# teamtomo/torch-motion-correction

Measured on AMD Instinct MI355X. Metric: frames/sec motion-corrected, 40×4k×4k fp32 stack, 1/2/4/8 MI355X, higher is better.
Workload: dtype f32; 1 GPU; 40-frame 4096x4096 fp32 movie, global rigid shift estimate+correct (estimate_global_motion -> correct_motion, frames + sum out), 1 stack per GPU per step, consecutive steps overlapped on two HIP streams; b_factor=500

## Files before the change

### torch_motion_correction_amd/csrc/mc_wave_fft.h

```cpp
#pragma once

#ifdef __HIPCC__
#include "mc_common.h"
#define MC_HD __host__ __device__ __forceinline__
#else
#include <math.h>
#include <stdint.h>
struct cfloat {
  float x, y;
};
#define MC_HD static inline
#endif

typedef float wf2 __attribute__((ext_vector_type(2)));

#define WF_N 2048
#define WF_SLAB 1024

MC_HD wf2 wf_make(float re, float im) { return wf2{re, im}; }
MC_HD wf2 wf_from(cfloat c) { return wf2{c.x, c.y}; }
MC_HD cfloat wf_to(wf2 v) { return cfloat{v.x, v.y}; }

MC_HD wf2 wf_add_mi(wf2 a, wf2 b) {
#if defined(__HIP_DEVICE_COMPILE__)
// ... 119 lines not shown
      a[4 * p + r] = a[4 * r + p];
      a[4 * r + p] = s;
    }
}

template <int KEEP>
MC_HD void wf_dft8_pruned(const wf2 (&e)[4], const wf2 (&o)[4], wf2 (&z)[8]) {
  const float H = 0.70710678118654752440f;
  wf2 e0 = e[0], e1 = e[1], e2 = e[2], e3 = e[3];
  wf2 o0 = o[0], o1 = o[1], o2 = o[2], o3 = o[3];
  wf_bfly4(e0, e1, e2, e3);
  wf_bfly4(o0, o1, o2, o3);
  z[0] = e0 + o0;
  z[7] = wf_fma_c(e3, o3, H, H);
  if (KEEP >= 2) {
    z[1] = wf_fma_c(e1, o1, H, -H);
    z[6] = wf_sub_mi(e2, o2);
  }
  if (KEEP >= 4) {
    z[2] = wf_add_mi(e2, o2);
    z[3] = wf_fma_c(e3, o3, -H, -H);
    z[4] = e0 - o0;
    z[5] = wf_fma_c(e1, o1, -H, H);
  }
}

struct WfLane {
  int x1w_base, x1w_mask;
  int x1r[4];
  int x2w;
  int x2r[4];
  int kbin[4];
  int self;
};

MC_HD WfLane wf_lane(int t) {
  WfLane L;
  {
    const int n2 = t >> 2, h1 = (t >> 1) & 1, h0 = t & 1;
    L.x1w_base = (n2 * 2 + h1) * 32 + h0 * 16;
    L.x1w_mask = (n2 & 3) | (h1 << 2) | (h0 << 3);
  }
  {
    const int k1 = t & 15, g2 = t >> 4, h1 = g2 >> 1, h0 = g2 & 1;
    const int lanepart = h1 * 32 + h0 * 16, lo = k1 ^ ((h1 << 2) | (h0 << 3));
    for (int v = 0; v < 4; ++v) L.x1r[v] = lanepart + (lo ^ v);
    L.x2w = g2 * 256 + k1;
  }
  L.kbin[0] = t;
  L.kbin[1] = t == 0 ? 128 : 256 - t;
  L.kbin[2] = 64 + t;
  L.kbin[3] = 192 - t;
  for (int s = 0; s < 4; ++s) L.x2r[s] = L.kbin[s];
  L.self = t == 0;
  return L;
}

MC_HD wf2 wf_unpack(wf2 zk, wf2 zmr, wf2 wk) {
  const wf2 zm = {zmr.x, -zmr.y};
  const wf2 sm = zk + zm, d = zk - zm;
  const wf2 wd = wf_cmul(d, wk);
  return wf_add_mi(sm, wd) * 0.5f;
}

template <int KEEP>
MC_HD void wf_unpack_lane(const wf2 (&z)[4][8], const wf2 (&wk)[4], bool self, wf2 (&X)[4][KEEP]) {
  const float C1 = 0.92387953251128673848f, S1 = 0.38268343236508978178f;
#pragma unroll
  for (int k3 = 0; k3 < KEEP; ++k3) {
    const wf2 m_a0 = self ? z[0][(8 - k3) & 7] : z[1][7 - k3];
    const wf2 m_a1 = self ? z[1][7 - k3] : z[0][7 - k3];
    wf2 w[4] = {wk[0], wk[1], wk[2], wk[3]};
    if (k3 == 1) {
#pragma unroll
      for (int s = 0; s < 4; ++s) w[s] = wf_cmulc(w[s], C1, -S1);
    }
    X[0][k3] = wf_unpack(z[0][k3], m_a0, w[0]);
    X[1][k3] = wf_unpack(z[1][k3], m_a1, w[1]);
    X[2][k3] = wf_unpack(z[2][k3], z[3][7 - k3], w[2]);
    X[3][k3] = wf_unpack(z[3][k3], z[2][7 - k3], w[3]);
  }
}

#define WF5_N 512
#define WF5_SLAB 512

MC_HD void wf_dft8(wf2 (&a)[8]) {
  const float H = 0.70710678118654752440f;
  wf2 e0 = a[0], e1 = a[2], e2 = a[4], e3 = a[6];
  wf2 o0 = a[1], o1 = a[3], o2 = a[5], o3 = a[7];
  wf_bfly4(e0, e1, e2, e3);
  wf_bfly4(o0, o1, o2, o3);
  a[0] = e0 + o0;
  a[4] = e0 - o0;
  a[1] = wf_fma_c(e1, o1, H, -H);
  a[5] = wf_fma_c(e1, o1, -H, H);
  a[2] = wf_add_mi(e2, o2);
  a[6] = wf_sub_mi(e2, o2);
  a[3] = wf_fma_c(e3, o3, -H, -H);
  a[7] = wf_fma_c(e3, o3, H, H);
}

MC_HD int wf5_x1(int k1, int n2, int n3) { return ((n2 * 8 + (k1 ^ n2)) * 8) + (n3 ^ (4 * (k1 >> 2))); }
MC_HD int wf5_x2(int k2, int n3, int k1) { return ((n3 * 8 + (k2 ^ n3)) * 8) + k1; }

#define WF10_N 1024
MC_HD int wf10_x1(int k1, int q) { return k1 * 64 + (q ^ ((2 * k1) & 31)); }
MC_HD int wf10_x2(int k1, int k2, int n3) { return n3 * 128 + k2 * 16 + k1; }

MC_HD void wf_twiddle8(wf2 (&a)[8], wf2 w1) {
  const wf2 w2 = wf_cmul(w1, w1), w3 = wf_cmul(w2, w1), w4 = wf_cmul(w2, w2);
  a[1] = wf_cmul(a[1], w1);
  a[2] = wf_cmul(a[2], w2);
  a[3] = wf_cmul(a[3], w3);
  a[4] = wf_cmul(a[4], w4);
  a[5] = wf_cmul(a[5], wf_cmul(w4, w1));
  a[6] = wf_cmul(a[6], wf_cmul(w4, w2));
  a[7] = wf_cmul(a[7], wf_cmul(w4, w3));
}
MC_HD void wf_twiddle16(wf2 (&a)[16], wf2 w1, wf2 w2, wf2 w4, wf2 w8) {
  const wf2 w3 = wf_cmul(w2, w1), w5 = wf_cmul(w4, w1), w6 = wf_cmul(w4, w2), w7 = wf_cmul(w4, w3);
  a[1] = wf_cmul(a[1], w1); a[2] = wf_cmul(a[2], w2); a[3] = wf_cmul(a[3], w3); a[4] = wf_cmul(a[4], w4);
  a[5] = wf_cmul(a[5], w5); a[6] = wf_cmul(a[6], w6); a[7] = wf_cmul(a[7], w7); a[8] = wf_cmul(a[8], w8);
  a[9] = wf_cmul(a[9], wf_cmul(w8, w1)); a[10] = wf_cmul(a[10], wf_cmul(w8, w2));
  a[11] = wf_cmul(a[11], wf_cmul(w8, w3)); a[12] = wf_cmul(a[12], wf_cmul(w8, w4));
  a[13] = wf_cmul(a[13], wf_cmul(w8, w5)); a[14] = wf_cmul(a[14], wf_cmul(w8, w6));
  a[15] = wf_cmul(a[15], wf_cmul(w8, w7));
}
```

### torch_motion_correction_amd/csrc/xc_fft.hip

```cpp
#include <stdlib.h>
#include <string.h>
#include <type_traits>
#include "xc_common.h"
#include "mc_wave_fft.h"




template <int LOGN, bool STATS, int RAW = 0>
__global__ __launch_bounds__(MC_WG) void xc_rows_fwd(
    const void* __restrict__ src_any, const int64_t* __restrict__ job_off, int64_t row_stride,
    const int* __restrict__ job_expo, const float* __restrict__ mask,
    const float* __restrict__ mean_rstd, cfloat* __restrict__ T1,
    const cfloat* __restrict__ tw_row, XcGeom g, XcBox box, double* __restrict__ stats_acc,
    const float* __restrict__ gain, const float* __restrict__ job_sub) {
  constexpr int N = 1 << LOGN;
  constexpr int NT = fft_threads(N), SG = MC_WG / NT;
  constexpr int R0 = FftPlan<N>::radix(0), NB0 = N / R0, IT0 = (NB0 + NT - 1) / NT;
  extern __shared__ __attribute__((aligned(16))) char smem[];
  const int tid = threadIdx.x;
  const int lt = tid & (NT - 1), sg = tid / NT;
  cfloat* l0 = reinterpret_cast<cfloat*>(smem) + sg * 2 * lds_len(N);
  cfloat* l1 = l0 + lds_len(N);
  cfloat* stg = reinterpret_cast<cfloat*>(smem) + SG * 2 * lds_len(N);
// ... 1169 lines not shown
    const cfloat* __restrict__ S_ref, const int* __restrict__ ref_idx, cfloat* __restrict__ T2n,
    float* __restrict__ bounds, const cfloat* __restrict__ tw_col, float scale, XcGeom g, int nstore) {
  constexpr int H = 1 << LOGH;
  __shared__ __attribute__((aligned(16))) cfloat line[R16 ? H : lds_len(H)];
  constexpr int NOUT = H / MC_WG;
  const int tid = threadIdx.x;
  const int p = blockIdx.y;
  const int nky = g.kyp + g.kyn;
  float acc[NOUT];
#pragma unroll
  for (int c = 0; c < NOUT; ++c) acc[c] = 0.f;
  const int64_t cur_base = (int64_t)cur_idx[p] * g.nkx, ref_base = (int64_t)ref_idx[p] * g.nkx;
  int kyi4[4];
  cfloat pc[4], pr[4];
  auto fetch4 = [&](int kx, cfloat (&c4)[4], cfloat (&r4)[4]) {
    const cfloat* cur = S_cur + (cur_base + kx) * nky;
    const cfloat* ref = S_ref + (ref_base + kx) * nky;
#pragma unroll
    for (int s4 = 0; s4 < 4; ++s4) {
      c4[s4] = kyi4[s4] >= 0 ? cur[kyi4[s4]] : cmake(0.f, 0.f);
      r4[s4] = kyi4[s4] >= 0 ? ref[kyi4[s4]] : cmake(0.f, 0.f);
    }
  };
  R16Tw TW;
  if constexpr (R16) {
    TW = r16_twiddles(tid, tw_col);
#pragma unroll
    for (int s4 = 0; s4 < 4; ++s4) kyi4[s4] = kept_index(tid + 256 * (s4 < 2 ? s4 : s4 + 12), H, g.kyp, g.kyn);
    if ((int)blockIdx.x * XC_NEAR_COLS < g.nkx) fetch4(blockIdx.x * XC_NEAR_COLS, pc, pr);
  }
#pragma unroll 1
  for (int cc = 0; cc < XC_NEAR_COLS; ++cc) {
    const int kx = blockIdx.x * XC_NEAR_COLS + cc;
    if (kx >= g.nkx) break;
    const cfloat* cur = S_cur + (cur_base + kx) * nky;
    const cfloat* ref = S_ref + (ref_base + kx) * nky;
    cfloat* outn = T2n + ((int64_t)p * g.nkx + kx) * (2 * nstore);
    const float wgt = kx == 0 ? 1.f : 2.f;
    auto load = [&](int ky) {
      const int kyi = kept_index(ky, H, g.kyp, g.kyn);
      if (kyi < 0) return cmake(0.f, 0.f);
      return cscale(cmulc(ref[kyi], cur[kyi]), scale);
    };
    cfloat qc[4], qr[4];
    if constexpr (R16) {
#pragma unroll
      for (int s4 = 0; s4 < 4; ++s4) {
        qc[s4] = pc[s4];
        qr[s4] = pr[s4];
      }
      if (cc + 1 < XC_NEAR_COLS && kx + 1 < g.nkx) fetch4(kx + 1, pc, pr);
    }
    auto load16 = [&](int n1, int) { return cscale(cmulc(qr[n1 < 2 ? n1 : n1 - 12], qc[n1 < 2 ? n1 : n1 - 12]), scale); };
    int c = 0;
    auto store = [&](int y, cfloat v) {
      const int yn = y < nstore ? y : y - (H - 2 * nstore);
      if (yn >= 0 && yn < 2 * nstore && (y < nstore || y >= H - nstore)) outn[yn] = v;
      acc[c++] += wgt * __builtin_amdgcn_sqrtf(v.x * v.x + v.y * v.y);
    };
    int tcol = tid;
    asm volatile("" : "+v"(tcol));
    __builtin_assume(tcol >= 0 && tcol < MC_WG);
    __builtin_assume(nstore > 0 && nstore <= 256);
    if constexpr (R16) wg_fft4096_r16_tw<+1, 2, 8>(line, tcol, TW, load16, store);
    else wg_fft<H, +1>(line, tcol, tw_col, 1, load, store);
    __syncthreads();
  }
  if constexpr (R16) {
#pragma unroll
    for (int k3 = 0; k3 < 16; ++k3) atomicAdd(&bounds[(int64_t)p * H + tid + 256 * k3], acc[k3]);
  } else {
    constexpr int R = (H >= 4096) ? 8 : (H == 2048 ? 4 : 2);
    constexpr int NB = H / R, IT = NB / MC_WG;
    static_assert(IT * R == NOUT, "row ownership of the last pass");
#pragma unroll
    for (int it = 0; it < IT; ++it)
#pragma unroll
      for (int m = 0; m < R; ++m)
        atomicAdd(&bounds[(int64_t)p * H + tid + it * MC_WG + m * NB], acc[it * R + m]);
  }
}

__global__ void xc_search_init(int* __restrict__ best, int* __restrict__ gate, float* __restrict__ bounds,
                               int npairs, int nbounds, float* __restrict__ shift_table, int nshift) {
  const int i = blockIdx.x * blockDim.x + threadIdx.x;
  if (i < nbounds) bounds[i] = 0.f;
  if (i < nshift) shift_table[i] = 0.f;
  if (i < npairs) best[i] = (int)0x807fffffu;
  if (i == 0) gate[0] = 0;
}

__global__ void xc_far_needed(const float* __restrict__ bounds, const int* __restrict__ best,
                              float* __restrict__ part_val, int* __restrict__ part_idx,
                              int* __restrict__ need_full, int H, int RG, int near) {
  const int ngrp = H / RG;
  const int p = blockIdx.y;
  const int grp = near + blockIdx.x * blockDim.x + threadIdx.x;
  if (grp >= ngrp - near) return;
  float b = 0.f;
  for (int r = 0; r < RG; ++r) b = fmaxf(b, bounds[(int64_t)p * H + grp * RG + r]);
  b = b * 1.0001f + 1e-30f;
  part_val[(int64_t)p * ngrp + grp] = -INFINITY;
  part_idx[(int64_t)p * ngrp + grp] = 0x7fffffff;
  const int fb = __float_as_int(b);
  if ((fb >= 0 ? fb : fb ^ 0x7fffffff) >= best[p]) atomicOr(need_full, 1);
}



__global__ __launch_bounds__(256) void xc_row_bounds(const cfloat* __restrict__ T2,
                                                     float* __restrict__ bounds, int nkx, int H) {
  __shared__ float part[4][64];
  const int ly = threadIdx.x & 63, slice = threadIdx.x >> 6;
  const int y = blockIdx.x * 64 + ly;
  const int p = blockIdx.y;
  float b0 = 0.f, b1 = 0.f, b2 = 0.f, b3 = 0.f;
  if (y < H) {
    const cfloat* in = T2 + (int64_t)p * nkx * H + y;
    int kx = slice;
    for (; kx + 12 < nkx; kx += 16) {
      const cfloat v0 = in[(int64_t)kx * H], v1 = in[(int64_t)(kx + 4) * H];
      const cfloat v2 = in[(int64_t)(kx + 8) * H], v3 = in[(int64_t)(kx + 12) * H];
      b0 += (kx == 0 ? 1.f : 2.f) * sqrtf(v0.x * v0.x + v0.y * v0.y);
      b1 += 2.f * sqrtf(v1.x * v1.x + v1.y * v1.y);
      b2 += 2.f * sqrtf(v2.x * v2.x + v2.y * v2.y);
      b3 += 2.f * sqrtf(v3.x * v3.x + v3.y * v3.y);
    }
    for (; kx < nkx; kx += 4) {
      const cfloat v = in[(int64_t)kx * H];
      b0 += (kx == 0 ? 1.f : 2.f) * sqrtf(v.x * v.x + v.y * v.y);
    }
  }
  part[slice][ly] = (b0 + b1) + (b2 + b3);
  __syncthreads();
  if (slice == 0 && y < H)
    bounds[(int64_t)p * H + y] = (part[0][ly] + part[1][ly]) + (part[2][ly] + part[3][ly]);
}

template <int LOGN, int EPI>
__global__ __launch_bounds__(MC_WG) void xc_rows_inv(const cfloat* __restrict__ T2,
                                                     const float* __restrict__ bounds,
                                                     int* __restrict__ best,
                                                     float* __restrict__ part_val,
                                                     int* __restrict__ part_idx,
                                                     float* __restrict__ out_real,
                                                     const int64_t* __restrict__ out_off,
                                                     int64_t out_stride,
                                                     const cfloat* __restrict__ tw_row, XcGeom g,
                                                     int near, int phase, int compact,
                                                     const int* __restrict__ gate) {
  constexpr int N = 1 << LOGN;
  if (gate && gate[0] == 0) return;
  constexpr int NT = fft_threads(N), SG = MC_WG / NT;
  constexpr int R0 = FftPlan<N>::radix(0), NB0 = N / R0, IT0 = (NB0 + NT - 1) / NT;
  extern __shared__ __attribute__((aligned(16))) char smem[];
  const int tid = threadIdx.x;
  const int lt = tid & (NT - 1), sg = tid / NT;
  cfloat* l0 = reinterpret_cast<cfloat*>(smem) + sg * 2 * lds_len(N);
  cfloat* l1 = l0 + lds_len(N);
  cfloat* stg = reinterpret_cast<cfloat*>(smem) + SG * 2 * lds_len(N);
  const int p = blockIdx.y;
  const int RG = g.RG;
  const int ngrp = g.H / RG;
  int grp = blockIdx.x;
  if (EPI == 0) grp = phase == 0 ? ((int)blockIdx.x < near ? (int)blockIdx.x : ngrp - 2 * near + (int)blockIdx.x)
                                 : near + (int)blockIdx.x;
  if constexpr (EPI == 0) {
    if (phase == 1) {
      float b = 0.f;
      for (int r = 0; r < RG; ++r) b = fmaxf(b, bounds[(int64_t)p * g.H + grp * RG + r]);
      b = b * 1.0001f + 1e-30f;
// ... 19 lines not shown
      const int kx = i / RG, r = i - kx * RG;
      if (i < g.nkx * RG) v8[u] = in[(int64_t)kx * cstride + r];
    }
#pragma unroll
    for (int u = 0; u < 8; ++u) {
      const int i = i0 + u * MC_WG;
      const int kx = i / RG, r = i - kx * RG;
      if (i < g.nkx * RG) stg[kx * (RG + 1) + r] = v8[u];
    }
  }
  FftTwiddles<N> T;
  T.template init<+1>(lt, tw_row, 2);
  cfloat wk[IT0][R0];
#pragma unroll
  for (int it = 0; it < IT0; ++it)
#pragma unroll
    for (int q = 0; q < R0; ++q) {
      const int j = lt + it * NT;
      const int k = (NB0 % NT == 0 || j < NB0) ? j + q * NB0 : 0;
      cfloat w = tw_row[k];
      w.y = -w.y;
      wk[it][q] = w;
    }
  __syncthreads();
  float bv = -INFINITY;
  int bi = 0x7fffffff;
  int s = 0;
  for (int r = sg; r < RG; r += SG) {
    const int y = grp * RG + r;
    auto load = [&](int k, int it, int q) {
      const int km = N - k;
      cfloat xk = (k < g.nkx) ? stg[k * (RG + 1) + r] : cmake(0.f, 0.f);
      cfloat xm = (km < g.nkx) ? cconj(stg[km * (RG + 1) + r]) : cmake(0.f, 0.f);
      if (k == 0) {
        xk.y = 0.f;
        xm.y = 0.f;
      }
      const cfloat sm = cadd(xk, xm), d = csub(xk, xm);
      const cfloat wd = cmul(wk[it][q], d);
      return cmake(sm.x - wd.y, sm.y + wd.x);
    };
    int res;
    if constexpr (EPI == 0) {
      auto store = [&](int n, cfloat v) {
        const int flat = y * g.W + 2 * n;
        cand_merge(bv, bi, v.x, flat);
        cand_merge(bv, bi, v.y, flat + 1);
      };
      res = wg_fft_pp<N, +1, true>(l0, l1, s, lt, T, load, store);
    } else {
      float* orow = out_real + out_off[p] + (int64_t)y * out_stride;
      auto store = [&](int n, cfloat v) {
        orow[2 * n] = v.x;
        orow[2 * n + 1] = v.y;
      };
      res = wg_fft_pp<N, +1, true>(l0, l1, s, lt, T, load, store);
    }
    s = res ^ 1;
  }
  if constexpr (EPI == 0) {
    for (int off = 32; off > 0; off >>= 1) {
      const float ov = __shfl_down(bv, off);
      const int oi = __shfl_down(bi, off);
      cand_merge(bv, bi, ov, oi);
    }
    __shared__ float wv[MC_WG / 64];
    __shared__ int wi[MC_WG / 64];
    if ((tid & 63) == 0) {
      wv[tid >> 6] = bv;
      wi[tid >> 6] = bi;
    }
    __syncthreads();
    if (tid == 0) {
      for (int w = 1; w < MC_WG / 64; ++w) cand_merge(bv, bi, wv[w], wi[w]);
      part_val[(int64_t)p * ngrp + grp] = bv;
      part_idx[(int64_t)p * ngrp + grp] = bi;
      atomicMax(&best[p], float_order(bv));
    }
  }
}

__global__ void xc_peak_final(const float* __restrict__ part_val, const int* __restrict__ part_idx,
                              int ngrp, int H, int W, int* __restrict__ peaks,
                              float* __restrict__ shifts, const int* __restrict__ shift_rows) {
  const int p = blockIdx.x;
  float bv = -INFINITY;
  int bi = 0x7fffffff;
  for (int i = threadIdx.x; i < ngrp; i += blockDim.x)
    cand_merge(bv, bi, part_val[(int64_t)p * ngrp + i], part_idx[(int64_t)p * ngrp + i]);
  for (int off = 32; off > 0; off >>= 1) {
    const float ov = __shfl_down(bv, off);
    const int oi = __shfl_down(bi, off);
    cand_merge(bv, bi, ov, oi);
  }
  if (threadIdx.x == 0) {
    if (bi == 0x7fffffff) bi = 0;
    peaks[p] = bi;
    const int py = bi / W, px = bi - py * W;
    const int row = shift_rows ? shift_rows[p] : p;
    shifts[2 * row] = (float)(py <= H / 2 ? py : py - H);
    shifts[2 * row + 1] = (float)(px <= W / 2 ? px : px - W);
  }
}

template <int LOGN>
__global__ __launch_bounds__(MC_WG) void xc_peak_nbhd(const cfloat* __restrict__ T2,
                                                      const int* __restrict__ peaks,
                                                      float* __restrict__ nb,
                                                      const cfloat* __restrict__ tw_row, XcGeom g,
                                                      const cfloat* __restrict__ T2n,
                                                      const int* __restrict__ gate, int nstore) {
  constexpr int N = 1 << LOGN;
  __shared__ __attribute__((aligned(16))) cfloat line[lds_len(N)];
  const int tid = threadIdx.x;
  const int p = blockIdx.y, dy = (int)blockIdx.x - 1;
  const int pk = peaks[p];
  const int py = pk / g.W, px = pk - py * g.W;
  const int y = py + dy;
  float* o = nb + (int64_t)p * 9 + (dy + 1) * 3;
  if (y < 0 || y >= g.H) {
    if (tid < 3) o[tid] = __builtin_nanf("");
    return;
  }
  const cfloat* in = T2 + (int64_t)p * g.nkx * g.H + y;
  int64_t cs = g.H;
  if (T2n && gate[0] == 0) {
    const int yn = y < nstore ? y : y - (g.H - 2 * nstore);
    if (yn < 0 || yn >= 2 * nstore || (y >= nstore && y < g.H - nstore)) {
      if (tid < 3) o[tid] = __builtin_nanf("");
      return;
    }
    cs = 2 * nstore;
    in = T2n + (int64_t)p * g.nkx * cs + yn;
  }
  auto X = [&](int k) { return in[(int64_t)k * cs]; };
  auto load = [&](int k) {
    const int km = N - k;
    cfloat xk = (k < g.nkx) ? X(k) : cmake(0.f, 0.f);
    cfloat xm = (km < g.nkx) ? cconj(X(km)) : cmake(0.f, 0.f);
    if (k == 0) {
      xk.y = 0.f;
      xm.y = 0.f;
    }
    const cfloat s = cadd(xk, xm), d = csub(xk, xm);
    cfloat w = tw_row[k];
    w.y = -w.y;
    const cfloat wd = cmul(w, d);
    return cmake(s.x - wd.y, s.y + wd.x);
  };
  auto store = [&](int n, cfloat v) { line[lpad(n)] = v; };
  wg_fft<N, +1>(line, tid, tw_row, 2, load, store);
  __syncthreads();
  if (tid < 3) {
    const int x = px + tid - 1;
    float v = __builtin_nanf("");
    if (x >= 0 && x < g.W) {
      const cfloat z = line[lpad(x >> 1)];
      v = (x & 1) ? z.y : z.x;
    }
    o[tid] = v;
  }
}

void mc_launch_row_bounds(const cfloat* T2, float* bounds, int nkx, int H, int npairs, hipStream_t stream) {
  hipLaunchKernelGGL(xc_row_bounds, dim3((H + 63) / 64, npairs), dim3(256), 0, stream, T2, bounds, nkx, H);
}
void mc_launch_peak_final(const float* part_val, const int* part_idx, int ngrp, int H, int W, int* peaks,
                          float* shifts, const int* shift_rows, int npairs, hipStream_t stream) {
  hipLaunchKernelGGL(xc_peak_final, dim3(npairs), dim3(64), 0, stream, part_val, part_idx, ngrp, H, W, peaks, shifts,
                     shift_rows);
}
#define MC_DISPATCH_LOG(LOGV, ...)          \
  switch (LOGV) {                           \
    MC_DISPATCH_CASE(4, __VA_ARGS__)        \
    MC_DISPATCH_CASE(5, __VA_ARGS__)        \
    MC_DISPATCH_CASE(6, __VA_ARGS__)        \
    MC_DISPATCH_CASE(7, __VA_ARGS__)        \
    MC_DISPATCH_CASE(8, __VA_ARGS__)        \
    MC_DISPATCH_CASE(9, __VA_ARGS__)        \
    MC_DISPATCH_CASE(10, __VA_ARGS__)       \
    MC_DISPATCH_CASE(11, __VA_ARGS__)       \
    MC_DISPATCH_CASE(12, __VA_ARGS__)       \
    default:                                \
      return MC_ERR_UNSUPPORTED;            \
  }


static int g_col_engine = 0;
static int g_row_engine = 0;
static bool mc_force_wg_rows() { return g_row_engine == 1; }
static bool mc_env_on(const char* name) {
  const char* v = getenv(name);
  return v && v[0] == '1';
}

static bool wave_rows_aligned(const float* src, const float* mask, int64_t row_stride) {
  return ((reinterpret_cast<uintptr_t>(src) | reinterpret_cast<uintptr_t>(mask)) & 15) == 0 &&
         (row_stride & 3) == 0;
}

static size_t rows_lds_bytes(int N, const XcGeom& g) {
  const int sgroups = MC_WG / fft_threads(N);
  return sizeof(cfloat) * ((size_t)sgroups * 2 * lds_len(N) + (size_t)g.nkx * (g.RG + 1));
}

extern "C" {

int mc_xc_col_engine(int mode) {
  if (mode < 0 || mode > 1) return MC_ERR_ARG;
  g_col_engine = mode;
  return MC_OK;
}

int mc_xc_row_engine(int mode) {
  if (mode < 0 || mode > 1) return MC_ERR_ARG;
  g_row_engine = mode;
  return MC_OK;
}

int mc_xc_rows_lds_bytes(const mc_xc_geom* q) {
  XcGeom g;
  int rc = geom_from(q, &g, true, false);
  if (rc) return rc;
  return (int)rows_lds_bytes(g.W / 2, g);
}

static int rows_forward_impl(const float* src, const int64_t* job_off, int64_t row_stride,
                             const int* job_expo, const float* mask, const float* mean_rstd,
                             void* T1, const void* tw_row, int njobs, const mc_xc_geom* q,
                             const XcBox* box, double* stats_acc, void* stream,
                             const int* row_chord = nullptr, bool half = false) {
  XcGeom g;
  int rc = geom_from(q, &g, true, false);
  if (rc) return rc;
  if (!src || !job_off || !T1 || !tw_row || njobs < 1) return MC_ERR_ARG;
  if (half && !(g.W == 2 * WF_N && g.nkx <= 512 && (g.ny % 8) == 0 && mask && !job_expo &&
                wave_rows_aligned(src, mask, row_stride) &&
                (!stats_acc || (((box ? box->wl : 0) | (box ? box->wu : 0)) & 255) == 0)))
    return MC_ERR_UNSUPPORTED;
  const int logn = mc_ilog2(g.W) - 1;
  XcBox b = box ? *box : XcBox{0, 0, 0, 0};
  if (g.W == 2 * WF_N && g.nkx <= 512 && (g.ny % 8) == 0 && mask && !job_expo &&
      wave_rows_aligned(src, mask, row_stride) && (!stats_acc || ((b.wl | b.wu) & 255) == 0) &&
      !mc_force_wg_rows()) {
    const int ngroups = (g.ny + WF_ROWS_PER_WG - 1) / WF_ROWS_PER_WG;
    dim3 grid((ngroups + 7) / 8 * 8, njobs);
    const size_t park_bytes = (size_t)4 * g.nkx * 16;
    const int lines16 = (WF_ROWS_PER_WG == 16 && mc_env_on("MC_K1_LINES16") && (g.ny % 16) == 0 && park_bytes <= 27 * 1024 &&
                         ((reinterpret_cast<uintptr_t>(T1) & 127) == 0)) ? 1 : 0;
    const size_t dyn = lines16 ? park_bytes : 0;
#define MC_WAVE_LAUNCH(KEEP, ST, LO, HI, CL, PF)                                                  \
  do {                                                                                            \
    auto kw = xc_rows_fwd_wave<KEEP, ST, LO, HI, CL, PF>;                                         \
// ... 275 lines not shown
                       const int* ref_idx, void* T2, const void* tw_col, float scale, int npairs,
                       const mc_xc_geom* q, void* stream) {
  XcGeom g;
  int rc = geom_from(q, &g, false, true);
  if (rc) return rc;
  if (!S_cur || !cur_idx || !S_ref || !ref_idx || !T2 || !tw_col || npairs < 1) return MC_ERR_ARG;
  if (g.H == 1024 && g.kyp <= 128 && g.kyn <= 128 && g_col_engine == 0) {
    hipLaunchKernelGGL(xc_cols_inv_wave1024, dim3((g.nkx + 3) / 4, npairs), dim3(256), 0, (hipStream_t)stream,
                       (const cfloat*)S_cur, cur_idx, (const cfloat*)S_ref, ref_idx, (cfloat*)T2,
                       (const cfloat*)tw_col, scale, g);
    return mc_check_launch();
  }
  dim3 grid(g.nkx, npairs);
  MC_DISPATCH_LOG(mc_ilog2(g.H), {
    hipLaunchKernelGGL((xc_cols_inv<L, 0>), grid, dim3(MC_WG), 0, (hipStream_t)stream,
                       (const cfloat*)S_cur, cur_idx, (const cfloat*)S_ref, ref_idx,
                       (const float*)nullptr, (cfloat*)T2, (const cfloat*)tw_col, scale, g,
                       (const int*)nullptr);
  });
  return mc_check_launch();
}

int mc_fourier_shift_cols_inverse(const void* S, const int* idx, const float* shifts, void* T2,
                                  const void* tw_col, float scale, int nframes,
                                  const mc_xc_geom* q, void* stream) {
  XcGeom g;
  int rc = geom_from(q, &g, false, true);
  if (rc) return rc;
  if (!S || !idx || !shifts || !T2 || !tw_col || nframes < 1) return MC_ERR_ARG;
  dim3 grid(g.nkx, nframes);
  MC_DISPATCH_LOG(mc_ilog2(g.H), {
    hipLaunchKernelGGL((xc_cols_inv<L, 1>), grid, dim3(MC_WG), 0, (hipStream_t)stream,
                       (const cfloat*)S, idx, (const cfloat*)nullptr, (const int*)nullptr, shifts,
                       (cfloat*)T2, (const cfloat*)tw_col, scale, g, (const int*)nullptr);
  });
  return mc_check_launch();
}

int mc_xc_rows_inverse_argmax(const void* T2, float* part_val, int* part_idx, int* peaks,
                              float* shifts, const void* tw_row, int npairs, const mc_xc_geom* q,
                              void* stream) {
  XcGeom g;
  int rc = geom_from(q, &g, true, false);
  if (rc) return rc;
  if (!T2 || !part_val || !part_idx || !peaks || !shifts || !tw_row || npairs < 1)
    return MC_ERR_ARG;
  const int logn = mc_ilog2(g.W) - 1;
  const size_t lds = rows_lds_bytes(g.W / 2, g);
  if (lds > 160 * 1024) return MC_ERR_ARG;
  const int ngrp = g.H / g.RG;
  int* best = part_idx + (int64_t)npairs * ngrp;
  {
    const float ninf = -INFINITY;
    int pat;
    memcpy(&pat, &ninf, 4);
    pat = pat >= 0 ? pat : pat ^ 0x7fffffff;
    hipError_t e = hipMemsetD32Async((hipDeviceptr_t)best, pat, npairs, (hipStream_t)stream);
    if (e != hipSuccess) return (int)e;
  }
  int near = (64 + g.RG - 1) / g.RG;
  if (2 * near > ngrp) near = ngrp / 2;
  float* bounds = part_val + (int64_t)npairs * ngrp;
  if (ngrp - 2 * near > 0)
    hipLaunchKernelGGL(xc_row_bounds, dim3((g.H + 63) / 64, npairs), dim3(256), 0, (hipStream_t)stream,
                       (const cfloat*)T2, bounds, g.nkx, g.H);
  MC_DISPATCH_LOG(logn, {
    auto k = xc_rows_inv<L, 0>;
    if (lds > 64 * 1024)
      (void)hipFuncSetAttribute((const void*)k, hipFuncAttributeMaxDynamicSharedMemorySize, (int)lds);
    if (near > 0)
      hipLaunchKernelGGL(k, dim3(2 * near, npairs), dim3(MC_WG), lds, (hipStream_t)stream,
                         (const cfloat*)T2, (const float*)bounds, best, part_val, part_idx, (float*)nullptr,
                         (const int64_t*)nullptr, (int64_t)0, (const cfloat*)tw_row, g, near, 0, 0,
                         (const int*)nullptr);
    if (ngrp - 2 * near > 0)
      hipLaunchKernelGGL(k, dim3(ngrp - 2 * near, npairs), dim3(MC_WG), lds, (hipStream_t)stream,
                         (const cfloat*)T2, (const float*)bounds, best, part_val, part_idx, (float*)nullptr,
                         (const int64_t*)nullptr, (int64_t)0, (const cfloat*)tw_row, g, near, 1, 0,
                         (const int*)nullptr);
  });
  rc = mc_check_launch();
  if (rc) return rc;
  hipLaunchKernelGGL(xc_peak_final, dim3(npairs), dim3(64), 0, (hipStream_t)stream, part_val,
                     part_idx, ngrp, g.H, g.W, peaks, shifts, (const int*)nullptr);
  return mc_check_launch();
}

int mc_xc_near_rows(const mc_xc_geom* q) {
  XcGeom g;
  int rc = geom_from(q, &g, true, true);
  if (rc) return rc;
  int near = (64 + g.RG - 1) / g.RG;
  if (2 * near > g.H / g.RG) near = (g.H / g.RG) / 2;
  return near * g.RG + XC_NEAR_GUARD;
}

int mc_xc_correlate_argmax(const void* S_cur, const int* cur_idx, const void* S_ref,
                           const int* ref_idx, void* T2_full, void* T2_near, float* part_val,
                           int* part_idx, int* peaks, float* shifts, const int* shift_rows,
                           int n_shift_rows, float* nb, const void* tw_col, const void* tw_row,
                           float scale, int npairs, const mc_xc_geom* q, void* stream) {
  XcGeom g;
  int rc = geom_from(q, &g, true, true);
  if (rc) return rc;
  if (!S_cur || !cur_idx || !S_ref || !ref_idx || !T2_full || !T2_near || !part_val || !part_idx ||
      !peaks || !shifts || !tw_col || !tw_row || npairs < 1)
    return MC_ERR_ARG;
  if (g.H < 1024) return MC_ERR_UNSUPPORTED;
  hipStream_t st = (hipStream_t)stream;
  const int logn = mc_ilog2(g.W) - 1;
  const size_t lds = rows_lds_bytes(g.W / 2, g);
  if (lds > 160 * 1024) return MC_ERR_ARG;
  const int ngrp = g.H / g.RG;
  int near = (64 + g.RG - 1) / g.RG;
  if (2 * near > ngrp) near = ngrp / 2;
  if (near < 1) return MC_ERR_UNSUPPORTED;
  const int nstore = near * g.RG + XC_NEAR_GUARD;
  if (nstore > 256) return MC_ERR_UNSUPPORTED;
  int* best = part_idx + (int64_t)npairs * ngrp;
  int* gate = best + npairs;
  float* bounds = part_val + (int64_t)npairs * ngrp;
  if (shift_rows && n_shift_rows < 1) return MC_ERR_ARG;
  hipLaunchKernelGGL(xc_search_init, dim3((npairs * g.H + 255) / 256), dim3(256), 0, st, best, gate, bounds,
                     npairs, npairs * g.H, shifts, shift_rows ? 2 * n_shift_rows : 0);
  if (g.H == 1024 && g.kyp <= 128 && g.kyn <= 128 && g_col_engine == 0) {
    hipLaunchKernelGGL(xc_cols_inv_near_wave1024, dim3((g.nkx + 4 * XC_NEAR_COLS_W - 1) / (4 * XC_NEAR_COLS_W), npairs),
                       dim3(256), 0, st, (const cfloat*)S_cur, cur_idx, (const cfloat*)S_ref, ref_idx,
                       (cfloat*)T2_near, bounds, (const cfloat*)tw_col, scale, g, nstore);
  } else if (g.H == 4096 && g.kyp <= 512 && g.kyn <= 512 && g_col_engine == 0) {
    hipLaunchKernelGGL((xc_cols_inv_near<12, true>), dim3((g.nkx + XC_NEAR_COLS - 1) / XC_NEAR_COLS, npairs),
                       dim3(MC_WG), 0, st, (const cfloat*)S_cur, cur_idx, (const cfloat*)S_ref, ref_idx,
                       (cfloat*)T2_near, bounds, (const cfloat*)tw_col, scale, g, nstore);
  } else
  MC_DISPATCH_LOG(mc_ilog2(g.H), {
    if constexpr (L >= 10) {
      hipLaunchKernelGGL(xc_cols_inv_near<L>, dim3((g.nkx + XC_NEAR_COLS - 1) / XC_NEAR_COLS, npairs),
                         dim3(MC_WG), 0, st, (const cfloat*)S_cur, cur_idx, (const cfloat*)S_ref, ref_idx,
                         (cfloat*)T2_near, bounds, (const cfloat*)tw_col, scale, g, nstore);
    } else {
      return MC_ERR_UNSUPPORTED;
    }
  });
  rc = mc_check_launch();
  if (rc) return rc;
  const int nfar = ngrp - 2 * near;
  MC_DISPATCH_LOG(logn, {
    auto k = xc_rows_inv<L, 0>;
    if (lds > 64 * 1024)
      (void)hipFuncSetAttribute((const void*)k, hipFuncAttributeMaxDynamicSharedMemorySize, (int)lds);
    hipLaunchKernelGGL(k, dim3(2 * near, npairs), dim3(MC_WG), lds, st, (const cfloat*)T2_near,
                       (const float*)bounds, best, part_val, part_idx, (float*)nullptr,
                       (const int64_t*)nullptr, (int64_t)0, (const cfloat*)tw_row, g, near, 0,
                       1 + XC_NEAR_GUARD, (const int*)nullptr);
  });
  rc = mc_check_launch();
  if (rc) return rc;
  if (nfar > 0) {
    hipLaunchKernelGGL(xc_far_needed, dim3((nfar + 63) / 64, npairs), dim3(64), 0, st,
                       (const float*)bounds, (const int*)best, part_val, part_idx, gate, g.H, g.RG, near);
    MC_DISPATCH_LOG(mc_ilog2(g.H), {
      hipLaunchKernelGGL((xc_cols_inv<L, 0>), dim3(g.nkx, npairs), dim3(MC_WG), 0, st,
                         (const cfloat*)S_cur, cur_idx, (const cfloat*)S_ref, ref_idx,
                         (const float*)nullptr, (cfloat*)T2_full, (const cfloat*)tw_col, scale, g,
                         (const int*)gate);
    });
    MC_DISPATCH_LOG(logn, {
      auto k = xc_rows_inv<L, 0>;
      hipLaunchKernelGGL(k, dim3(nfar, npairs), dim3(MC_WG), lds, st, (const cfloat*)T2_full,
                         (const float*)bounds, best, part_val, part_idx, (float*)nullptr,
                         (const int64_t*)nullptr, (int64_t)0, (const cfloat*)tw_row, g, near, 1, 0,
                         (const int*)gate);
    });
    rc = mc_check_launch();
    if (rc) return rc;
  }
  hipLaunchKernelGGL(xc_peak_final, dim3(npairs), dim3(64), 0, st, part_val, part_idx, ngrp, g.H, g.W,
                     peaks, shifts, shift_rows);
  if (nb) {
    MC_DISPATCH_LOG(logn, {
      hipLaunchKernelGGL(xc_peak_nbhd<L>, dim3(3, npairs), dim3(MC_WG), 0, st, (const cfloat*)T2_full,
                         (const int*)peaks, nb, (const cfloat*)tw_row, g, (const cfloat*)T2_near,
                         (const int*)gate, nstore);
    });
  }
  return mc_check_launch();
}

int mc_xc_rows_inverse_store(const void* T2, float* out, const int64_t* out_off,
                             int64_t out_stride, const void* tw_row, int nframes,
                             const mc_xc_geom* q, void* stream) {
  XcGeom g;
  int rc = geom_from(q, &g, true, false);
  if (rc) return rc;
  if (!T2 || !out || !out_off || !tw_row || nframes < 1) return MC_ERR_ARG;
  const int logn = mc_ilog2(g.W) - 1;
  const size_t lds = rows_lds_bytes(g.W / 2, g);
  if (lds > 160 * 1024) return MC_ERR_ARG;
  dim3 grid(g.H / g.RG, nframes);
  MC_DISPATCH_LOG(logn, {
    auto k = xc_rows_inv<L, 1>;
    if (lds > 64 * 1024)
      (void)hipFuncSetAttribute((const void*)k, hipFuncAttributeMaxDynamicSharedMemorySize, (int)lds);
    hipLaunchKernelGGL(k, grid, dim3(MC_WG), lds, (hipStream_t)stream, (const cfloat*)T2,
                       (const float*)nullptr, (int*)nullptr, (float*)nullptr, (int*)nullptr, out, out_off, out_stride,
                       (const cfloat*)tw_row, g, 0, 0, 0, (const int*)nullptr);
  });
  return mc_check_launch();
}

int mc_xc_peak_neighbourhood(const void* T2, const int* peaks, float* nb, const void* tw_row,
                             int npairs, const mc_xc_geom* q, void* stream) {
  XcGeom g;
  int rc = geom_from(q, &g, true, false);
  if (rc) return rc;
  if (!T2 || !peaks || !nb || !tw_row || npairs < 1) return MC_ERR_ARG;
  const int logn = mc_ilog2(g.W) - 1;
  dim3 grid(3, npairs);
  MC_DISPATCH_LOG(logn, {
    hipLaunchKernelGGL(xc_peak_nbhd<L>, grid, dim3(MC_WG), 0, (hipStream_t)stream,
                       (const cfloat*)T2, peaks, nb, (const cfloat*)tw_row, g, (const cfloat*)nullptr,
                       (const int*)nullptr, 0);
  });
  return mc_check_launch();
}

}
```

Baseline: 24670 frames/s.

## Add wave-level pruned inverse row FFT with fused last-block far-gate and peak finalize

Adds a new xc_rows_inv_wave kernel that runs the near-band inverse row FFTs of the cross-correlation with one wavefront per row. It uses a pruned real-output pass, where only KEEP input bins are nonzero, and takes its twiddles from an LDS table. The last block, found through an atomic ticket, does the work of xc_far_needed and writes peaks and shifts itself. xc_peak_final is then skipped when the gate is closed. This is meant to remove launches and the generic workgroup FFT cost on the 4096-wide path, at the price of extra atomics, threadfences and new correctness risk in the ticket logic.

```diff
diff --git a/torch_motion_correction_amd/csrc/mc_wave_fft.h b/torch_motion_correction_amd/csrc/mc_wave_fft.h
--- a/torch_motion_correction_amd/csrc/mc_wave_fft.h
+++ b/torch_motion_correction_amd/csrc/mc_wave_fft.h
@@ -225,6 +225,71 @@
   }
 }
 
+
+MC_HD void wfi_pack(wf2 X, wf2 w, wf2& zk, wf2& zm) {
+  const wf2 R = {X.x * w.x + X.y * w.y, X.y * w.x - X.x * w.y};
+  zk = wf2{X.y + R.x, X.x - R.y};
+  zm = wf2{R.x - X.y, R.y + X.x};
+}
+
+template <int KEEP>
+MC_HD void wf_dft8_lo(const wf2 (&z)[8], wf2 (&y)[8]) {
+  const float H = 0.70710678118654752440f;
+  if (KEEP == 1) {
+    const wf2 a = z[0], b = z[7];
+    y[0] = a + b;
+    y[1] = wf_fma_c(a, b, H, H);
+    y[2] = wf_sub_mi(a, b);
+    y[3] = wf_fma_c(a, b, -H, H);
+    y[4] = a - b;
+    y[5] = wf_fma_c(a, b, -H, -H);
+    y[6] = wf_add_mi(a, b);
+    y[7] = wf_fma_c(a, b, H, -H);
+  } else {
+    const wf2 e0 = z[0] + z[6], e1 = wf_sub_mi(z[0], z[6]), e2 = z[0] - z[6], e3 = wf_add_mi(z[0], z[6]);
+    const wf2 o0 = z[1] + z[7], o1 = wf_sub_mi(z[1], z[7]), o2 = z[1] - z[7], o3 = wf_add_mi(z[1], z[7]);
+    y[0] = e0 + o0;
+    y[4] = e0 - o0;
+    y[1] = wf_fma_c(e1, o1, H, -H);
+    y[5] = wf_fma_c(e1, o1, -H, H);
+    y[2] = wf_add_mi(e2, o2);
+    y[6] = wf_sub_mi(e2, o2);
+    y[3] = wf_fma_c(e3, o3, -H, -H);
+    y[7] = wf_fma_c(e3, o3, H, H);
+  }
+}
+
+template <int KEEP>
+MC_HD void wfi_pass_c(const wf2 (&X)[4][KEEP], const wf2 (&wk)[4], bool self, wf2 (&y)[4][8]) {
+  const float C1 = 0.92387953251128673848f, S1 = 0.38268343236508978178f;
+  wf2 zk[4][KEEP], zm[4][KEEP];
+#pragma unroll
+  for (int s = 0; s < 4; ++s)
+#pragma unroll
+    for (int k3 = 0; k3 < KEEP; ++k3)
+      wfi_pack(X[s][k3], k3 == 1 ? wf_cmulc(wk[s], C1, -S1) : wk[s], zk[s][k3], zm[s][k3]);
+  const wf2 zero = {0.f, 0.f};
+  wf2 z[4][8];
+#pragma unroll
+  for (int k3 = 0; k3 < KEEP; ++k3) {
+    z[0][k3] = zk[0][k3];
+    z[1][k3] = zk[1][k3];
+    z[2][k3] = zk[2][k3];
+    z[3][k3] = zk[3][k3];
+    const wf2 own = k3 + 1 < KEEP ? zm[0][k3 + 1] : zero;
+    z[0][7 - k3] = self ? own : zm[1][k3];
+    z[1][7 - k3] = self ? zm[1][k3] : zm[0][k3];
+    z[2][7 - k3] = zm[3][k3];
+    z[3][7 - k3] = zm[2][k3];
+  }
+#pragma unroll
+  for (int s = 0; s < 4; ++s) {
+#pragma unroll
+    for (int i = KEEP; i < 8 - KEEP; ++i) z[s][i] = zero;
+    wf_dft8_lo<KEEP>(z[s], y[s]);
+  }
+}
+
 #define WF5_N 512
 #define WF5_SLAB 512
 
diff --git a/torch_motion_correction_amd/csrc/xc_fft.hip b/torch_motion_correction_amd/csrc/xc_fft.hip
--- a/torch_motion_correction_amd/csrc/xc_fft.hip
+++ b/torch_motion_correction_amd/csrc/xc_fft.hip
@@ -1275,11 +1275,13 @@
 }
 
 __global__ void xc_search_init(int* __restrict__ best, int* __restrict__ gate, float* __restrict__ bounds,
-                               int npairs, int nbounds, float* __restrict__ shift_table, int nshift) {
+                               int npairs, int nbounds, float* __restrict__ shift_table, int nshift,
+                               int* __restrict__ ticket, int tstride) {
   const int i = blockIdx.x * blockDim.x + threadIdx.x;
   if (i < nbounds) bounds[i] = 0.f;
   if (i < nshift) shift_table[i] = 0.f;
   if (i < npairs) best[i] = (int)0x807fffffu;
+  if (ticket && i < npairs) ticket[(int64_t)i * tstride] = 0;
   if (i == 0) gate[0] = 0;
 }
 
@@ -1465,7 +1467,9 @@
 
 __global__ void xc_peak_final(const float* __restrict__ part_val, const int* __restrict__ part_idx,
                               int ngrp, int H, int W, int* __restrict__ peaks,
-                              float* __restrict__ shifts, const int* __restrict__ shift_rows) {
+                              float* __restrict__ shifts, const int* __restrict__ shift_rows,
+                              const int* __restrict__ gate) {
+  if (gate && gate[0] == 0) return;
   const int p = blockIdx.x;
   float bv = -INFINITY;
   int bi = 0x7fffffff;
@@ -1483,6 +1487,203 @@
     const int row = shift_rows ? shift_rows[p] : p;
     shifts[2 * row] = (float)(py <= H / 2 ? py : py - H);
     shifts[2 * row + 1] = (float)(px <= W / 2 ? px : px - W);
+  }
+}
+
+#define WFI_TAB (WF_TWA + WF_TWB + 256)
+template <int KEEP>
+__global__ __launch_bounds__(1024) void xc_rows_inv_wave(
+    const cfloat* __restrict__ T2n, const float* __restrict__ bounds, int* __restrict__ best,
+    float* __restrict__ part_val, int* __restrict__ part_idx, int* __restrict__ gate,
+    int* __restrict__ peaks, float* __restrict__ shifts, const int* __restrict__ shift_rows,
+    const cfloat* __restrict__ tw_row, XcGeom g, int near, int guard) {
+  extern __shared__ __attribute__((aligned(16))) cfloat wfi_slabs[];
+  __shared__ __attribute__((aligned(16))) cfloat tab[WFI_TAB];
+  __shared__ float red_v[16];
+  __shared__ int red_i[16];
+  __shared__ int is_last;
+  const cfloat* twA = tab;
+  const cfloat* twB = tab + WF_TWA;
+  const cfloat* twK = tab + WF_TWA + WF_TWB;
+  const int tid = threadIdx.x, nthr = blockDim.x;
+  const int t = tid & 63;
+  const int wv = __builtin_amdgcn_readfirstlane(tid >> 6);
+  const int p = blockIdx.y;
+  const int RG = g.RG, lrg = 31 - __builtin_clz(RG);
+  const int ngrp = g.H / RG;
+  const int grp = (int)blockIdx.x < near ? (int)blockIdx.x : ngrp - 2 * near + (int)blockIdx.x;
+  const int nstore = near * RG + guard, cstride = 2 * nstore;
+  const int coff = (int)blockIdx.x < near ? (int)blockIdx.x * RG : nstore + guard + ((int)blockIdx.x - near) * RG;
+  const cfloat* in = T2n + (int64_t)p * g.nkx * cstride + coff;
+  {
+    cfloat v8[8];
+    for (int i0 = tid; i0 < g.nkx * RG; i0 += 8 * nthr) {
+#pragma unroll
+      for (int u = 0; u < 8; ++u) {
+        const int i = i0 + u * nthr;
+        const int kx = i >> lrg, r = i & (RG - 1);
+        if (i < g.nkx * RG) v8[u] = in[(int64_t)kx * cstride + r];
+      }
+#pragma unroll
+      for (int u = 0; u < 8; ++u) {
+        const int i = i0 + u * nthr;
+        const int kx = i >> lrg, r = i & (RG - 1);
+        if (i < g.nkx * RG) wfi_slabs[r * WF_SLAB + kx + r] = v8[u];
+      }
+    }
+  }
+  for (int i = tid; i < WFI_TAB; i += nthr) {
+    int src_k;
+    if (i < WF_TWA) {
+      src_k = (2 * (i & 127)) << (i >> 7);
+    } else if (i < WF_TWA + WF_TWB) {
+      const int e = i - WF_TWA, h = e & 1, k2 = ((e >> 1) % 15) + 1, gq = e / 30;
+      src_k = 32 * (2 * gq + h) * k2;
+    } else {
+      const int e = i - WF_TWA - WF_TWB, sl = e >> 6, l = e & 63;
+      src_k = sl == 0 ? l : (sl == 1 ? (l == 0 ? 128 : 256 - l) : (sl == 2 ? 64 + l : 192 - l));
+    }
+    tab[i] = tw_row[src_k];
+  }
+  __syncthreads();
+  wf2* slab = reinterpret_cast<wf2*>(wfi_slabs + wv * WF_SLAB);
+  const WfLane L = wf_lane(t);
+  wf2 Y[4][8];
+  {
+    wf2 X[4][KEEP], wk[4];
+#pragma unroll
+    for (int s = 0; s < 4; ++s) {
+      wk[s] = wf_from(twK[64 * s + t]);
+#pragma unroll
+      for (int k3 = 0; k3 < KEEP; ++k3) {
+        const int k = L.kbin[s] + 256 * k3;
+        X[s][k3] = k < g.nkx ? slab[k + wv] : wf2{0.f, 0.f};
+        if (s == 0 && k3 == 0 && t == 0) X[s][k3].y = 0.f;
+      }
+    }
+    wf_sync();
+    wfi_pass_c<KEEP>(X, wk, L.self != 0, Y);
+  }
+  wf2 B0[16], B1[16];
+#pragma unroll
+  for (int s = 0; s < 4; ++s)
+#pragma unroll
+    for (int n3h = 0; n3h < 4; ++n3h) slab[L.x2r[s] + 256 * n3h] = Y[s][2 * n3h];
+  wf_sync();
+#pragma unroll
+  for (int k2 = 0; k2 < 16; ++k2) B0[k2] = slab[L.x2w + 16 * k2];
+  wf_sync();
+#pragma unroll
+  for (int s = 0; s < 4; ++s)
+#pragma unroll
+    for (int n3h = 0; n3h < 4; ++n3h) slab[L.x2r[s] + 256 * n3h] = Y[s][2 * n3h + 1];
+  wf_sync();
+#pragma unroll
+  for (int k2 = 0; k2 < 16; ++k2) B1[k2] = slab[L.x2w + 16 * k2];
+  wf_sync();
+  {
+    const float4* twb = reinterpret_cast<const float4*>(twB) + (t >> 4) * 15;
+#pragma unroll
+    for (int k2 = 1; k2 < 16; ++k2) {
+      const float4 w = twb[k2 - 1];
+      B0[k2] = wf_cmul(B0[k2], wf2{w.x, w.y});
+      B1[k2] = wf_cmul(B1[k2], wf2{w.z, w.w});
+    }
+  }
+  wf2 A0[16], A1[16];
+  wf_dft16(B0);
+#pragma unroll
+  for (int n2 = 0; n2 < 16; ++n2) slab[L.x1r[n2 & 3] + 64 * n2] = B0[n2];
+  wf_sync();
+#pragma unroll
+  for (int k1 = 0; k1 < 16; ++k1) A0[k1] = slab[L.x1w_base + (k1 ^ L.x1w_mask)];
+  wf_sync();
+  wf_dft16(B1);
+#pragma unroll
+  for (int n2 = 0; n2 < 16; ++n2) slab[L.x1r[n2 & 3] + 64 * n2] = B1[n2];
+  wf_sync();
+#pragma unroll
+  for (int k1 = 0; k1 < 16; ++k1) A1[k1] = slab[L.x1w_base + (k1 ^ L.x1w_mask)];
+  float bv = -INFINITY;
+  int bi = 0x7fffffff;
+  {
+    const float4* twa = reinterpret_cast<const float4*>(twA) + t;
+    float4 w[4];
+#pragma unroll
+    for (int sb = 0; sb < 4; ++sb) w[sb] = twa[sb * 64];
+    const int flat0 = (grp * RG + wv) * g.W + 4 * t;
+    wf_twiddle16(A0, wf2{w[0].x, w[0].y}, wf2{w[1].x, w[1].y}, wf2{w[2].x, w[2].y}, wf2{w[3].x, w[3].y});
+    wf_dft16(A0);
+#pragma unroll
+    for (int n1 = 0; n1 < 16; ++n1) {
+      cand_merge(bv, bi, A0[n1].y, flat0 + 256 * n1);
+      cand_merge(bv, bi, A0[n1].x, flat0 + 256 * n1 + 1);
+    }
+    wf_twiddle16(A1, wf2{w[0].z, w[0].w}, wf2{w[1].z, w[1].w}, wf2{w[2].z, w[2].w}, wf2{w[3].z, w[3].w});
+    wf_dft16(A1);
+#pragma unroll
+    for (int n1 = 0; n1 < 16; ++n1) {
+      cand_merge(bv, bi, A1[n1].y, flat0 + 256 * n1 + 2);
+      cand_merge(bv, bi, A1[n1].x, flat0 + 256 * n1 + 3);
+    }
+  }
+  for (int off = 32; off > 0; off >>= 1) {
+    const float ov = __shfl_down(bv, off);
+    const int oi = __shfl_down(bi, off);
+    cand_merge(bv, bi, ov, oi);
+  }
+  if (t == 0) {
+    red_v[wv] = bv;
+    red_i[wv] = bi;
+  }
+  __syncthreads();
+  int* ticket = part_idx + (int64_t)p * ngrp + near;
+  if (tid == 0) {
+    for (int w = 1; w < RG; ++w) cand_merge(bv, bi, red_v[w], red_i[w]);
+    __hip_atomic_store(reinterpret_cast<int*>(&part_val[(int64_t)p * ngrp + grp]), __float_as_int(bv), __ATOMIC_RELAXED,
+                       __HIP_MEMORY_SCOPE_AGENT);
+    __hip_atomic_store(&part_idx[(int64_t)p * ngrp + grp], bi, __ATOMIC_RELAXED, __HIP_MEMORY_SCOPE_AGENT);
+    atomicMax(&best[p], float_order(bv));
+    __threadfence();
+    is_last = atomicAdd(ticket, 1) == 2 * near - 1;
+  }
+  __syncthreads();
+  if (!is_last) return;
+  __threadfence();
+  const int bestp = __hip_atomic_load(&best[p], __ATOMIC_RELAXED, __HIP_MEMORY_SCOPE_AGENT);
+  int open = 0;
+  for (int fg = near + tid; fg < ngrp - near; fg += nthr) {
+    float b = 0.f;
+    for (int r = 0; r < RG; ++r) b = fmaxf(b, bounds[(int64_t)p * g.H + fg * RG + r]);
+    b = b * 1.0001f + 1e-30f;
+    part_val[(int64_t)p * ngrp + fg] = -INFINITY;
+    part_idx[(int64_t)p * ngrp + fg] = 0x7fffffff;
+    if (float_order(b) >= bestp) open = 1;
+  }
+  if (open) atomicOr(gate, 1);
+  if (tid < 64) {
+    bv = -INFINITY;
+    bi = 0x7fffffff;
+    for (int i = tid; i < 2 * near; i += 64) {
+      const int ng = i < near ? i : ngrp - 2 * near + i;
+      const int vi = __hip_atomic_load(reinterpret_cast<int*>(&part_val[(int64_t)p * ngrp + ng]), __ATOMIC_RELAXED,
+                                       __HIP_MEMORY_SCOPE_AGENT);
+      const int ii = __hip_atomic_load(&part_idx[(int64_t)p * ngrp + ng], __ATOMIC_RELAXED, __HIP_MEMORY_SCOPE_AGENT);
+      cand_merge(bv, bi, __int_as_float(vi), ii);
+    }
+    for (int off = 32; off > 0; off >>= 1) {
+      const float ov = __shfl_down(bv, off);
+      const int oi = __shfl_down(bi, off);
+      cand_merge(bv, bi, ov, oi);
+    }
+    if (tid == 0) {
+      if (bi == 0x7fffffff) bi = 0;
+      peaks[p] = bi;
+      const int py = bi / g.W, px = bi - py * g.W;
+      const int row = shift_rows ? shift_rows[p] : p;
+      shifts[2 * row] = (float)(py <= g.H / 2 ? py : py - g.H);
+      shifts[2 * row + 1] = (float)(px <= g.W / 2 ? px : px - g.W);
+    }
   }
 }
 
@@ -1551,7 +1752,7 @@
 void mc_launch_peak_final(const float* part_val, const int* part_idx, int ngrp, int H, int W, int* peaks,
                           float* shifts, const int* shift_rows, int npairs, hipStream_t stream) {
   hipLaunchKernelGGL(xc_peak_final, dim3(npairs), dim3(64), 0, stream, part_val, part_idx, ngrp, H, W, peaks, shifts,
-                     shift_rows);
+                     shift_rows, (const int*)nullptr);
 }
 #define MC_DISPATCH_LOG(LOGV, ...)          \
   switch (LOGV) {                           \
@@ -1993,7 +2194,7 @@
   rc = mc_check_launch();
   if (rc) return rc;
   hipLaunchKernelGGL(xc_peak_final, dim3(npairs), dim3(64), 0, (hipStream_t)stream, part_val,
-                     part_idx, ngrp, g.H, g.W, peaks, shifts, (const int*)nullptr);
+                     part_idx, ngrp, g.H, g.W, peaks, shifts, (const int*)nullptr, (const int*)nullptr);
   return mc_check_launch();
 }
 
@@ -2032,8 +2233,12 @@
   int* gate = best + npairs;
   float* bounds = part_val + (int64_t)npairs * ngrp;
   if (shift_rows && n_shift_rows < 1) return MC_ERR_ARG;
+  const int nfar = ngrp - 2 * near;
+  const bool wave_near = g.W == 4096 && g.nkx <= 512 && !nb && !mc_force_wg_rows() && nfar > 0 && g.RG <= 16 &&
+                         mc_is_pow2(g.RG);
   hipLaunchKernelGGL(xc_search_init, dim3((npairs * g.H + 255) / 256), dim3(256), 0, st, best, gate, bounds,
-                     npairs, npairs * g.H, shifts, shift_rows ? 2 * n_shift_rows : 0);
+                     npairs, npairs * g.H, shifts, shift_rows ? 2 * n_shift_rows : 0,
+                     wave_near ? part_idx + near : (int*)nullptr, ngrp);
   if (g.H == 1024 && g.kyp <= 128 && g.kyn <= 128 && g_col_engine == 0) {
     hipLaunchKernelGGL(xc_cols_inv_near_wave1024, dim3((g.nkx + 4 * XC_NEAR_COLS_W - 1) / (4 * XC_NEAR_COLS_W), npairs),
                        dim3(256), 0, st, (const cfloat*)S_cur, cur_idx, (const cfloat*)S_ref, ref_idx,
@@ -2054,7 +2259,18 @@
   });
   rc = mc_check_launch();
   if (rc) return rc;
-  const int nfar = ngrp - 2 * near;
+  if (wave_near) {
+    const size_t wlds = (size_t)g.RG * WF_SLAB * sizeof(cfloat);
+    auto launch = [&](auto k) {
+      if (wlds > 48 * 1024)
+        (void)hipFuncSetAttribute((const void*)k, hipFuncAttributeMaxDynamicSharedMemorySize, (int)wlds);
+      hipLaunchKernelGGL(k, dim3(2 * near, npairs), dim3(64 * g.RG), wlds, st, (const cfloat*)T2_near,
+                         (const float*)bounds, best, part_val, part_idx, gate, peaks, shifts, shift_rows,
+                         (const cfloat*)tw_row, g, near, XC_NEAR_GUARD);
+    };
+    if (g.nkx <= 256) launch(xc_rows_inv_wave<1>);
+    else launch(xc_rows_inv_wave<2>);
+  } else
   MC_DISPATCH_LOG(logn, {
     auto k = xc_rows_inv<L, 0>;
     if (lds > 64 * 1024)
@@ -2067,8 +2283,9 @@
   rc = mc_check_launch();
   if (rc) return rc;
   if (nfar > 0) {
-    hipLaunchKernelGGL(xc_far_needed, dim3((nfar + 63) / 64, npairs), dim3(64), 0, st,
-                       (const float*)bounds, (const int*)best, part_val, part_idx, gate, g.H, g.RG, near);
+    if (!wave_near)
+      hipLaunchKernelGGL(xc_far_needed, dim3((nfar + 63) / 64, npairs), dim3(64), 0, st,
+                         (const float*)bounds, (const int*)best, part_val, part_idx, gate, g.H, g.RG, near);
     MC_DISPATCH_LOG(mc_ilog2(g.H), {
       hipLaunchKernelGGL((xc_cols_inv<L, 0>), dim3(g.nkx, npairs), dim3(MC_WG), 0, st,
                          (const cfloat*)S_cur, cur_idx, (const cfloat*)S_ref, ref_idx,
@@ -2086,7 +2303,7 @@
     if (rc) return rc;
   }
   hipLaunchKernelGGL(xc_peak_final, dim3(npairs), dim3(64), 0, st, part_val, part_idx, ngrp, g.H, g.W,
-                     peaks, shifts, shift_rows);
+                     peaks, shifts, shift_rows, wave_near ? (const int*)gate : (const int*)nullptr);
   if (nb) {
     MC_DISPATCH_LOG(logn, {
       hipLaunchKernelGGL(xc_peak_nbhd<L>, dim3(3, npairs), dim3(MC_WG), 0, st, (const cfloat*)T2_full,
```

Result: slower. 22480 frames/s (-8.9%).
